# bobhansky/WhittedStyle_Raytracer

Hardware: NVIDIA B200
Metric: Mrays/s (all ray types), out/water_bunny_tex.txt + shadow soft @ 3840x2160 (higher is better)
Workload: dtype f32

## Files before the change

### include/wrt_cuda.h

```cpp
#ifndef WRT_CUDA_H
#define WRT_CUDA_H

#include "wrt_scene.h"

#ifdef __cplusplus
extern "C" {
#endif

typedef struct WrtContext WrtContext;

#define WRT_TRAVERSAL_EXHAUSTIVE 0
#define WRT_TRAVERSAL_PRUNED     1


int  wrt_create(int device, WrtContext** out);
void wrt_destroy(WrtContext* ctx);
const char* wrt_last_error(void);

int wrt_upload_scene(WrtContext* ctx, const WrtSceneDesc* scene);
int wrt_set_camera(WrtContext* ctx, const WrtCamera* cam);

int wrt_set_tiles(WrtContext* ctx, int tile_w, int tile_h, int rank, int world);

int wrt_set_options(WrtContext* ctx, int traversal, uint32_t seed, float queue_factor);

int wrt_enable_kernel_timing(WrtContext* ctx, int on);

int wrt_trace_closest(WrtContext* ctx, const float* orig, const float* dir, int64_t n, WrtHit* hits);
int wrt_trace_closest_wavefront(WrtContext* ctx, const float* orig, const float* dir, int64_t n, WrtHit* hits);
int wrt_shadow_hard(WrtContext* ctx, const float* pos, const float* ndir, const float* lightpos, int64_t n, float* coeff);
int wrt_shadow_soft(WrtContext* ctx, const float* pos, const float* ndir, const float* lightpos, int64_t n, float* coeff);
int wrt_shadow_directional(WrtContext* ctx, const float* pos, const int32_t* self_object, const float* lightdir4,
                           int64_t n, float* coeff);

int wrt_render(WrtContext* ctx, uint8_t* rgb_host, WrtStats* stats);

int wrt_render_device(WrtContext* ctx, void* d_rgb_tiles, void* cuda_stream);
int wrt_finish_device(WrtContext* ctx, WrtStats* stats);
int wrt_get_stats(WrtContext* ctx, WrtStats* stats);

int64_t wrt_tile_pixel_count(WrtContext* ctx, int rank, int world);

int wrt_scatter_tiles(WrtContext* ctx, const void* d_gathered, int world, int64_t stride_bytes,
                      void* d_rgb_image, void* cuda_stream);

int64_t wrt_kernel_launch_count(WrtContext* ctx);

int wrt_measure_fp32_peak(WrtContext* ctx, float* tflops_fma, float* tflops_mul_add);

#define WRT_KERNEL_FAMILIES 11
int wrt_get_kernel_times(WrtContext* ctx, float* ms, int capacity);
int wrt_get_kernel_launches(WrtContext* ctx, int32_t* launches, int capacity);

typedef struct WrtMulti WrtMulti;
int  wrt_multi_create(const int* devices, int n, WrtMulti** out);
void wrt_multi_destroy(WrtMulti* m);
int  wrt_multi_device_count(WrtMulti* m);
WrtContext* wrt_multi_context(WrtMulti* m, int rank);
int  wrt_multi_uses_peer_stores(WrtMulti* m);
int  wrt_multi_upload_scene(WrtMulti* m, const WrtSceneDesc* scene);
int  wrt_multi_set_camera(WrtMulti* m, const WrtCamera* cam);
int  wrt_multi_set_options(WrtMulti* m, int traversal, uint32_t seed, float queue_factor);
int  wrt_multi_render(WrtMulti* m, uint8_t* rgb_host, WrtStats* stats);

#ifdef __cplusplus
}
#endif
#endif
```

### whittedstyle_raytracer_b200/csrc/cuda/kernels.cuh

```cuda
#pragma once
#include <cooperative_groups.h>

#include "dev_shade.cuh"
#include "shaft_cull.h"
#include "../../../include/wrt_rng.h"
#include "../../../include/wrt_tiles.h"

#ifdef WRT_MIN_BLOCKS
#define WRT_TRACE_BOUNDS __launch_bounds__(128, WRT_MIN_BLOCKS)
#else
#define WRT_TRACE_BOUNDS __launch_bounds__(128)
#endif
#ifndef WRT_TRACE_DEEP_STEPS
#define WRT_TRACE_DEEP_STEPS 8
#endif
namespace wrt {

#ifdef WRT_DEBUG_BOUNDS
__device__ unsigned g_wrt_bounds_line = 0;
__device__ __forceinline__ bool wrt_bounds_ok(bool ok, unsigned line) {
    if (!ok) atomicCAS(&g_wrt_bounds_line, 0u, line);
    return ok;
}
#define WRT_IN_BOUNDS(idx, cap) wrt_bounds_ok((unsigned long long)(idx) < (unsigned long long)(cap), (unsigned)__LINE__)
#else
#define WRT_IN_BOUNDS(idx, cap) true
#endif

enum CounterSlot {
    C_NRAYS = 0,
    C_NTRAYS = 112,
    C_NPREQ = 16,
    C_NDREQ = 32,
    C_VALID0 = 48,
    C_OVERFLOW = 49,
    C_NEMPTY = 50,
    C_NCULL = 128,
    C_NSKIP = 144,
    C_NDSKIP = 160,
    C_POOL = 176,
    C_NWORK = 180,
    C_WORK = 192,
    C_TOTAL = 256
};

struct TileMap : WrtTileMap {
    __host__ __device__ bool slot_to_pixel(long long slot, int rank_, int& px, int& py) const {
        return wrt_tilemap_slot_to_pixel(this, slot, rank_, &px, &py) != 0;
    }
};

#define WRT_QUEUES 3

struct PrimaryGen {
    WrtCamera cam;
    TileMap tm;
    long long slot0;
};

struct FrameBuffers {
    float4* ray_o[2];
    float4* ray_d[2];
    float4* hit;
    float4* surf;
    float4* node_a;
    float4* node_b;
    float4* preq_o[WRT_QUEUES];
    uint4*  preq_k[WRT_QUEUES];
    float4* dreq_o[WRT_QUEUES];
    uint4*  dreq_k[WRT_QUEUES];
    unsigned char queue_of_level[WRT_MAX_DEPTH + 3];
    float*  coeff;
    unsigned* counters;
    unsigned cap0, capd;
    unsigned preq_cap[WRT_QUEUES], dreq_cap[WRT_QUEUES];
    unsigned n_node_cap;
};

__device__ __forceinline__ unsigned node_id(const FrameBuffers& fb, int level, unsigned slot) {
    return level == 0 ? slot : fb.cap0 + (unsigned)(level - 1) * fb.capd + slot;
}

__device__ __forceinline__ unsigned warp_alloc(unsigned* counter, int k, unsigned cap, unsigned* overflow) {
    unsigned lane = threadIdx.x & 31;
    int incl = k;
#pragma unroll
    for (int off = 1; off < 32; off <<= 1) {
        int n = __shfl_up_sync(0xffffffffu, incl, off);
        if (lane >= (unsigned)off) incl += n;
    }
    int total = __shfl_sync(0xffffffffu, incl, 31);
    unsigned base = 0;
    if (lane == 31 && total > 0) base = atomicAdd(counter, (unsigned)total);
    base = __shfl_sync(0xffffffffu, base, 31);
    unsigned mine = base + (unsigned)(incl - k);
    if (k > 0 && (mine > cap || (unsigned)k > cap - mine)) { *overflow = 1u; return 0xffffffffu; }
    return mine;
}

struct LevelSpan {
    unsigned nR, nT, half;
    __device__ __forceinline__ unsigned count() const { return nR + nT; }
    __device__ __forceinline__ unsigned slot(unsigned item) const { return item < nR ? item : half + (item - nR); }
};
__device__ __forceinline__ LevelSpan level_span(const FrameBuffers& fb, int level, unsigned n0) {
    LevelSpan sp;
    if (level == 0) {
        sp.half = fb.cap0; sp.nT = 0;
        sp.nR = n0 < fb.cap0 ? n0 : fb.cap0;
    } else {
        const unsigned* counters = fb.counters;
        sp.half = fb.capd / 2;
        sp.nR = counters[C_NRAYS + level] < sp.half ? counters[C_NRAYS + level] : sp.half;
        sp.nT = counters[C_NTRAYS + level] < fb.capd - sp.half ? counters[C_NTRAYS + level] : fb.capd - sp.half;
    }
    return sp;
}

__device__ __forceinline__ unsigned queue_len(const unsigned* counters, int slot, unsigned cap) {
    unsigned n = counters[slot];
    return n < cap ? n : cap;
}

__device__ __forceinline__ bool primary_ray(const PrimaryGen& pg, unsigned item, f3& org, f3& dir, unsigned& pixel) {
    const WrtCamera& cam = pg.cam;
    int x, y;
    if (!pg.tm.slot_to_pixel(pg.slot0 + item, pg.tm.rank, x, y)) {
        org = mk3(0.f, 0.f, 0.f); dir = mk3(0.f, 0.f, 1.f); pixel = 0xffffffffu;
        return false;
    }
    f3 ul = mk3(cam.ul[0], cam.ul[1], cam.ul[2]);
    f3 v_off = (float)y * mk3(cam.delta_v[0], cam.delta_v[1], cam.delta_v[2]);
    f3 h_off = (float)x * mk3(cam.delta_h[0], cam.delta_h[1], cam.delta_h[2]);
    f3 pixelPos = ul + h_off + v_off + mk3(cam.c_off_h[0], cam.c_off_h[1], cam.c_off_h[2]) +
                  mk3(cam.c_off_v[0], cam.c_off_v[1], cam.c_off_v[2]);
    f3 eye = mk3(cam.eye[0], cam.eye[1], cam.eye[2]);
    f3 nrm = mk3(cam.n[0], cam.n[1], cam.n[2]);
    if (!cam.parallel) { dir = normalized(pixelPos - eye); org = eye; }
    else { dir = nrm; org = pixelPos - cam.d * nrm; }
    pixel = (unsigned)(y * cam.width + x);
    return true;
}

#define WRT_CULL_UNLIT 1
#define WRT_CULL_SHAFT 2
__device__ __forceinline__ void surface_warp(const DevScene& s, const FrameBuffers& fb, int level, int cull, bool live,
                                             f3 org, f3 dir, unsigned pixel, unsigned path, float hit_t, int prim,
                                             float b1, float b2, unsigned slot) {
    const unsigned child_half = fb.capd / 2;
    const int q = fb.queue_of_level[level];
    float4* nray_o = fb.ray_o[(level + 1) & 1];
// ... 155 lines not shown
            unsigned pixel;
            if (!primary_ray(pg, (unsigned)item, o, d, pixel)) { cs.best.prim = -2; return false; }
        } else {
            o = mk3(ray_o[idx]); d = mk3(ray_d[idx]);
        }
        if (s.n_nodes == 0) return false;
        r = make_ray(o, d);
        float prune = prune_cfg;
        const bool ref_tree = prune < 0.f || degenerate_dir(r.d);
        if (ref_tree) prune = -1.f;
        const size_t oct_off = (size_t)ray_octant(r.d) * 2 * (size_t)s.n_nodes;
        nodes = (ref_tree ? s.ronodes : s.onodes) + oct_off;
        cs.set_ray(s, r, prune);
        float te;
        float4 lo = ldg4(nodes), hi = ldg4(nodes + 1);
        if (!slab_presorted(lo, hi, r, te)) return false;
        cur = __float_as_int(lo.w);
        if (cur < 0) { cs.leaf(s, r, ~cur); return false; }
        wide = WRT_WIDE4 && !LEVEL0 && !ref_tree;
        if (wide) nodes = s.wnodes + (WRT_WIDE_FLOAT4_PER_RECORD / 2) * oct_off;
        return true;
    }
    __device__ __forceinline__ bool step(int& cur, Stack& st) {
#if WRT_LEAF_DEFER
        if (WRT_WIDE4 && !LEVEL0 && wide) return traverse_step4_defer<true>(nodes, r, st, cur, cs.limit, [&](int p) { cs.leaf(s, r, p); });
#else
        if (WRT_WIDE4 && !LEVEL0 && wide) return traverse_step4<true>(nodes, r, st, cur, cs.limit, [&](int p) { cs.leaf(s, r, p); });
#endif
        return traverse_step<true, true>(nodes, r, st, cur, cs.limit, [&](int p) { cs.leaf(s, r, p); });
    }
    __device__ __forceinline__ bool finish(int&, Stack&) {
        if (WRT_IN_BOUNDS(idx, fb.cap0 > fb.capd ? fb.cap0 : fb.capd))
            fb.hit[idx] = make_float4(cs.best.t, __int_as_float(cs.best.prim), cs.best.u, cs.best.v);
        return false;
    }
};

template <bool LEVEL0>
__global__ void WRT_TRACE_BOUNDS k_trace_closest(const __grid_constant__ DevScene s, const __grid_constant__ FrameBuffers fb,
                                                 const __grid_constant__ PrimaryGen pg, int level, unsigned n0, int work_slot,
                                                 float prune_rel, int refill) {
    extern __shared__ int smem[];
    Stack st;
    st.init(smem, threadIdx.x, blockDim.x);
    ClosestQuery<LEVEL0> q(s, fb, pg, level, n0, prune_rel);
    run_queue<ClosestQuery<LEVEL0>, LEVEL0 ? WRT_STEPS_PER_ROUND : WRT_TRACE_DEEP_STEPS>(
        q, q.span.count(), reinterpret_cast<unsigned long long*>(fb.counters + work_slot), st, refill);
}

#ifndef WRT_SURFACE_MIN_BLOCKS
#define WRT_SURFACE_MIN_BLOCKS 4
#endif
__global__ void __launch_bounds__(256, WRT_SURFACE_MIN_BLOCKS) k_surface_spawn(const __grid_constant__ DevScene s, const __grid_constant__ FrameBuffers fb,
                                                       const __grid_constant__ PrimaryGen pg, int level, unsigned n0, int cull) {
    const LevelSpan span = level_span(fb, level, n0);
    const unsigned n = span.count();
    const unsigned n_round = (n + 31u) & ~31u;
    unsigned valid = 0;
    for (unsigned item = blockIdx.x * blockDim.x + threadIdx.x; item < n_round; item += gridDim.x * blockDim.x) {
        const bool live = item < n;
        const unsigned i = span.slot(live ? item : 0);
        f3 org = mk3(0.f, 0.f, 0.f), dir = org;
        unsigned pixel = 0, path = 0;
        float4 h = make_float4(0.f, __int_as_float(-2), 0.f, 0.f);
        if (live) {
            h = fb.hit[i];
            if (level == 0) {
                path = 1u;
                if (primary_ray(pg, item, org, dir, pixel)) ++valid;
            } else {
                float4 o4 = fb.ray_o[level & 1][i], d4 = fb.ray_d[level & 1][i];
                org = mk3(o4); dir = mk3(d4);
                pixel = __float_as_uint(o4.w); path = __float_as_uint(d4.w);
            }
        }
        surface_warp(s, fb, level, cull, live, org, dir, pixel, path, h.x, __float_as_int(h.y), h.z, h.w, i);
    }
    if (level == 0) {
        valid = __reduce_add_sync(0xffffffffu, valid);
        if ((threadIdx.x & 31) == 0 && valid) atomicAdd(fb.counters + C_VALID0, valid);
    }
}

struct HardShadowQuery {
    const DevScene& s;
    const FrameBuffers& fb;
    Ray r;
    const float4* nodes;
    float dis;
    ShadowAcc acc;
    size_t out;
    int q;
    bool wide;
    bool literal;
    __device__ __forceinline__ HardShadowQuery(const DevScene& s_, const FrameBuffers& fb_, int q_, bool literal_)
        : s(s_), fb(fb_), q(q_), literal(literal_) {}
    __device__ __forceinline__ bool begin(unsigned long long item, int& cur, Stack&) {
        float4 o4 = fb.preq_o[q][item];
        uint4 k = fb.preq_k[q][item];
        const WrtLight* L = s.lights + k.x;
        f3 orig = mk3(o4);
        f3 lightPos = mk3(L->pos[0], L->pos[1], L->pos[2]);
        f3 raydir = normalized(lightPos - orig);
        dis = norm(lightPos - orig);
        r = make_ray(orig, raydir);
        out = (size_t)__float_as_uint(o4.w) * (unsigned)s.n_lights + k.x;
        acc.reset();
        if (s.n_nodes == 0) return false;
        const bool ref_tree = literal || degenerate_dir(raydir);
        const size_t oct_off = (size_t)ray_octant(raydir) * 2 * (size_t)s.n_nodes;
        nodes = (ref_tree ? s.ronodes : s.onodes) + oct_off;
        float te;
        float4 lo = ldg4(nodes), hi = ldg4(nodes + 1);
        if (!slab_presorted(lo, hi, r, te)) return false;
        cur = __float_as_int(lo.w);
        if (cur < 0) { shadow_leaf(s, r, dis, ~cur, acc); return false; }
        wide = WRT_WIDE4 && !ref_tree;
        if (wide) nodes = s.wnodes + (WRT_WIDE_FLOAT4_PER_RECORD / 2) * oct_off;
        return true;
    }
    __device__ __forceinline__ bool step(int& cur, Stack& st) {
        const float never = INFINITY;
        bool more;
#if WRT_LEAF_DEFER >= 2
        if (WRT_WIDE4 && wide) more = traverse_step4_defer<false>(nodes, r, st, cur, never, [&](int p) { shadow_leaf(s, r, dis, p, acc); });
#else
        if (WRT_WIDE4 && wide) more = traverse_step4<false>(nodes, r, st, cur, never, [&](int p) { shadow_leaf(s, r, dis, p, acc); });
#endif
        else more = traverse_step<false, true>(nodes, r, st, cur, never, [&](int p) { shadow_leaf(s, r, dis, p, acc); });
        return more && acc.res != 0.f;
    }
    __device__ __forceinline__ bool finish(int&, Stack&) {
        const float v = shadow_value(s, acc);
        if (WRT_IN_BOUNDS(out, (size_t)fb.n_node_cap * s.n_lights)) fb.coeff[out] = v;
        return false;
    }
};

__global__ void WRT_TRACE_BOUNDS k_shadow_hard(const __grid_constant__ DevScene s, const __grid_constant__ FrameBuffers fb, int q, int work_slot, int refill,
                                               int literal) {
    extern __shared__ int smem[];
    Stack st;
    st.init(smem, threadIdx.x, blockDim.x);
    const unsigned n = queue_len(fb.counters, C_NPREQ + q, fb.preq_cap[q]);
    HardShadowQuery hq(s, fb, q, literal != 0);
    run_queue(hq, n, reinterpret_cast<unsigned long long*>(fb.counters + work_slot), st, refill);
}

struct SoftShadowQuery {
    const DevScene& s;
    const FrameBuffers& fb;
    unsigned seed;
    Ray r;
    const float4* nodes;
    float dis;
    bool occ;
    size_t out;
    int q;
    int last_occ;
    bool use_cache;
    __device__ __forceinline__ SoftShadowQuery(const DevScene& s_, const FrameBuffers& fb_, unsigned seed_, int q_, bool cache)
        : s(s_), fb(fb_), seed(seed_), q(q_), last_occ(-1), use_cache(cache && !s_.has_light_prims) {}
    __device__ __forceinline__ bool begin(unsigned long long item, int& cur, Stack& st) {
        unsigned req = (unsigned)(item / WRT_SOFT_SAMPLES);
        unsigned sample = (unsigned)(item - (unsigned long long)req * WRT_SOFT_SAMPLES);
        float4 o4 = fb.preq_o[q][req];
// ... 832 lines not shown
```

### whittedstyle_raytracer_b200/csrc/cuda/ploc_bvh.h

```cpp
#ifndef WRT_PLOC_BVH_H
#define WRT_PLOC_BVH_H

#include <math.h>
#include <stdint.h>

#ifdef __CUDACC__
#define WRT_PLOC_HD __host__ __device__ __forceinline__
#else
#include <vector_types.h>
#include <vector_functions.h>
#define WRT_PLOC_HD static inline
#endif

#define WRT_PLOC_RADIUS 8

struct PlocTree {
    float4* lo;
    float4* hi;
    float4* dlo;
    float4* dhi;
    int* parent;
    int* cnt;
};

WRT_PLOC_HD float ploc_fmin(float a, float b) { return a < b ? a : b; }
WRT_PLOC_HD float ploc_fmax(float a, float b) { return a > b ? a : b; }
WRT_PLOC_HD int ploc_f2i(float f) { union { float f; int i; } u; u.f = f; return u.i; }
WRT_PLOC_HD float ploc_i2f(int i) { union { float f; int i; } u; u.i = i; return u.f; }

WRT_PLOC_HD uint64_t ploc_expand21(uint64_t v) {
    v &= 0x1fffffull;
    v = (v | v << 32) & 0x1f00000000ffffull;
    v = (v | v << 16) & 0x1f0000ff0000ffull;
    v = (v | v << 8) & 0x100f00f00f00f00full;
    v = (v | v << 4) & 0x10c30c30c30c30c3ull;
    v = (v | v << 2) & 0x1249249249249249ull;
    return v;
}
WRT_PLOC_HD uint64_t ploc_morton(const float c[3], const float bmin[3], const float bmax[3]) {
    uint64_t code = 0;
    for (int k = 0; k < 3; k++) {
        float ext = bmax[k] - bmin[k];
        float t = ext > 0.f ? (c[k] - bmin[k]) / ext : 0.f;
        if (!(t > 0.f)) t = 0.f;
        if (t > 1.f) t = 1.f;
        uint64_t q = (uint64_t)(t * 2097151.0f);
        code |= ploc_expand21(q) << k;
    }
    return code;
}

WRT_PLOC_HD void ploc_init_leaf(const PlocTree& t, int p, const float mn[3], const float mx[3], float dil_rel, float dil_abs) {
    t.lo[p] = make_float4(mn[0], mn[1], mn[2], ploc_i2f(-1));
    t.hi[p] = make_float4(mx[0], mx[1], mx[2], ploc_i2f(-1));
    float ext = 0.f;
    for (int k = 0; k < 3; k++) {
        ext = ploc_fmax(ext, mx[k] - mn[k]);
        ext = ploc_fmax(ext, ploc_fmax(fabsf(mn[k]), fabsf(mx[k])) * 1e-2f);
    }
    const float pad = dil_rel * ext + dil_abs;
    t.dlo[p] = make_float4(mn[0] - pad, mn[1] - pad, mn[2] - pad, 0.f);
    t.dhi[p] = make_float4(mx[0] + pad, mx[1] + pad, mx[2] + pad, 0.f);
    t.parent[p] = -1;
    t.cnt[p] = 1;
}

WRT_PLOC_HD float ploc_union_area(const float4 alo, const float4 ahi, const float4 blo, const float4 bhi) {
    float dx = ploc_fmax(ahi.x, bhi.x) - ploc_fmin(alo.x, blo.x);
    float dy = ploc_fmax(ahi.y, bhi.y) - ploc_fmin(alo.y, blo.y);
    float dz = ploc_fmax(ahi.z, bhi.z) - ploc_fmin(alo.z, blo.z);
    return dx * dy + dy * dz + dz * dx;
}

WRT_PLOC_HD bool ploc_tie_before(int i, int j, int k) {
    const bool jb = j == (i ^ 1), kb = k == (i ^ 1);
    if (jb != kb) return jb;
    const int dj = j > i ? j - i : i - j, dk = k > i ? k - i : i - k;
    if (dj != dk) return dj < dk;
    return (j < i ? j : i) < (k < i ? k : i);
}
WRT_PLOC_HD int ploc_nearest(const PlocTree& t, const int* cl, int m, int i, int radius) {
    const int a = cl[i];
    const float4 alo = t.lo[a], ahi = t.hi[a];
    float best = INFINITY;
    int bj = -1;
    const int j0 = i - radius > 0 ? i - radius : 0, j1 = i + radius < m - 1 ? i + radius : m - 1;
    for (int j = j0; j <= j1; j++) {
        if (j == i) continue;
        const int b = cl[j];
        float d = ploc_union_area(alo, ahi, t.lo[b], t.hi[b]);
        if (!(d == d)) d = INFINITY;
        if (bj < 0 || d < best || (d == best && ploc_tie_before(i, j, bj))) { best = d; bj = j; }
    }
    return bj;
}

WRT_PLOC_HD int ploc_fate(const int* nn, int i) {
    const int j = nn[i];
    if (j < 0 || nn[j] != i) return 1;
    return i < j ? 2 : 0;
}

WRT_PLOC_HD void ploc_make_node(const PlocTree& t, int id, int a, int b) {
    const float4 alo = t.lo[a], ahi = t.hi[a], blo = t.lo[b], bhi = t.hi[b];
    t.lo[id] = make_float4(ploc_fmin(alo.x, blo.x), ploc_fmin(alo.y, blo.y), ploc_fmin(alo.z, blo.z), ploc_i2f(a));
    t.hi[id] = make_float4(ploc_fmax(ahi.x, bhi.x), ploc_fmax(ahi.y, bhi.y), ploc_fmax(ahi.z, bhi.z), ploc_i2f(b));
    const float4 dal = t.dlo[a], dah = t.dhi[a], dbl = t.dlo[b], dbh = t.dhi[b];
    t.dlo[id] = make_float4(ploc_fmin(dal.x, dbl.x), ploc_fmin(dal.y, dbl.y), ploc_fmin(dal.z, dbl.z), 0.f);
    t.dhi[id] = make_float4(ploc_fmax(dah.x, dbh.x), ploc_fmax(dah.y, dbh.y), ploc_fmax(dah.z, dbh.z), 0.f);
    t.cnt[id] = t.cnt[a] + t.cnt[b];
    t.parent[id] = -1;
    t.parent[a] = id;
    t.parent[b] = id;
}

WRT_PLOC_HD int ploc_record_of(const PlocTree& t, int n_leaves, int v, int* link, int* depth) {
    int acc = 0, d = 0, own_extra = 0, own_right = 0;
    int u = v;
    while (t.parent[u] >= 0) {
        const int p = t.parent[u];
        const int left = ploc_f2i(t.lo[p].w);
        const int right = u != left;
        const int extra = 2 + (right ? 2 * t.cnt[left] - 2 : 0);
        if (u == v) { own_extra = extra; own_right = right; }
        acc += extra;
        u = p;
        ++d;
    }
    *depth = d;
    const int F = 2 + acc;
    *link = v < n_leaves ? ~v : F;
    return d == 0 ? 0 : F - own_extra + own_right;
// ... 4 lines not shown
```

### whittedstyle_raytracer_b200/csrc/cuda/wrt_cuda.cu

```cuda
#include <algorithm>
#include <cstdio>
#include <chrono>
#include <cstdlib>
#include <cstring>
#include <condition_variable>
#include <functional>
#include <mutex>
#include <string>
#include <thread>
#include <vector>

#include <cuda_runtime.h>

#include "../../../include/wrt_cuda.h"
#include "fast_bvh.hpp"
#include "kernels.cuh"
#include "bvh_build.cuh"

namespace {

thread_local std::string g_err;

int fail(const std::string& msg) {
    g_err = msg;
    return 1;
}

#define CK(call)                                                                                      \
    do {                                                                                              \
        cudaError_t e_ = (call);                                                                      \
        if (e_ != cudaSuccess) {                                                                      \
            return fail(std::string(#call) + ": " + cudaGetErrorString(e_) + " (" + __FILE__ + ":" + \
                        std::to_string(__LINE__) + ")");                                              \
        }                                                                                             \
    } while (0)

enum Family { F_RAYGEN, F_TRACE, F_SURFACE, F_SHADOW_HARD, F_SHADOW_SOFT, F_SHADOW_DIR, F_SHADE, F_COMBINE, F_RESOLVE, F_SOFT_LISTS, F_SOFT_FILTER };

struct TimedLaunch {
    int family;
    cudaEvent_t e0, e1;
    bool on_chain;
};

}

struct WrtContext {
    int device = 0;
    int num_sms = 0;
    cudaStream_t chain = nullptr, side = nullptr;
    cudaEvent_t ev_in = nullptr, ev_lvl0 = nullptr, ev_mid = nullptr, ev_side = nullptr, ev_out = nullptr;
    bool overlap = true;

    wrt::DevScene ds{};
    std::vector<void*> scene_allocs;
    std::vector<size_t> scene_alloc_bytes;
    size_t scene_slot = 0;
    bool has_scene = false;
    bool textures_complete = true;
    int bvh_depth = 0;
    int stack_rows = 2;
    std::vector<WrtPathCode> path_codes;

    WrtCamera cam{};
    bool has_cam = false;
    int tile_w = 8, tile_h = 4, rank = 0, world = 1;
    int traversal = WRT_TRAVERSAL_PRUNED;
    uint32_t seed = WRT_DEFAULT_SEED;
    float queue_factor = 0.f;
    float deep_factor = 0.25f;
    float prune_rel = 1e-3f;
    bool kernel_timing = false;
    int refill = 16;
    int refill_soft = 24;
    bool shaft_cull = true;
    bool soft_lists = true;
    long long list_pool_cap_override = 0;
    int shaft_cull_max_level = 0;
    wrt::SoftListBuffers list_bufs[WRT_QUEUES] = {};
    wrt::FastBvhBuilder fbvh;
    bool host_bvh = false;
    uint8_t* h_stage = nullptr;
    size_t h_stage_bytes = 0;
    int ploc_coop_grid = 1;
    int fast_depth = 0, build_passes = 0;
    bool unlit_cull = true;
    int cache_from_level = 0;
    int chunk_div = 16;
    int refill0 = 32;
    int trace_blocks_per_sm = 10;
    bool shade0_separate = true;
    int soft_filter = 2;
    int deep_split = 5;
    int side_blocks_per_sm = 6;
    int fb_split = -1;
    bool small_batch_full_levels = true;
    long long max_batch = 1ll << 25;
    long long learned_batch = 1ll << 40;
    long long learned_key[4] = {0, 0, 0, 0};

    wrt::FrameBuffers fb{};
    std::vector<void*> frame_allocs;
    unsigned batch_slots = 0;
    unsigned deep_slots = 0;
    int fb_lights = -1, fb_point = -1, fb_dir = -1;
    unsigned* h_counters = nullptr;
    uint8_t* d_image = nullptr;
    size_t d_image_bytes = 0;
    uint8_t* h_image = nullptr;
    size_t h_image_bytes = 0;

    void* d_scratch[5] = {nullptr, nullptr, nullptr, nullptr, nullptr};
    size_t scratch_bytes[5] = {0, 0, 0, 0, 0};

    int64_t launches = 0;
    int work_seq = 0;
    int coop_grid = 0;
    int filter_grid = 0;
    WrtStats stats{};
    std::vector<TimedLaunch> timed;
    std::vector<cudaEvent_t> event_pool;
    size_t event_next = 0;
    float family_ms[WRT_KERNEL_FAMILIES] = {0};
    int family_launches[WRT_KERNEL_FAMILIES] = {0};
    cudaEvent_t ev_begin = nullptr, ev_end = nullptr;
    cudaStream_t user_stream = nullptr;
    bool user_stream_joined = false;
    uint8_t* last_image = nullptr;
    uint8_t* last_packed = nullptr;
    bool frame_pending = false;
    bool has_frame = false;

    wrt::TileMap tilemap() const {
        wrt::TileMap tm;
        static_cast<WrtTileMap&>(tm) = wrt_tilemap_make(cam.width, cam.height, tile_w, tile_h, rank, world);
        return tm;
    }
    long long local_slots(int r, int w) const {
        WrtTileMap tm = wrt_tilemap_make(cam.width, cam.height, tile_w, tile_h, r, w);
        return wrt_tilemap_slots(&tm, r, w);
    }
};

namespace {

using wrt::FrameBuffers;

int dev_alloc(WrtContext* c, size_t bytes, void** out) {
    *out = nullptr;
    bytes = std::max<size_t>(bytes, 256);
    size_t slot = c->scene_slot++;
    if (slot >= c->scene_allocs.size()) { c->scene_allocs.push_back(nullptr); c->scene_alloc_bytes.push_back(0); }
    if (c->scene_alloc_bytes[slot] < bytes) {
        if (c->scene_allocs[slot]) {
            CK(cudaDeviceSynchronize());
            cudaFree(c->scene_allocs[slot]);
        }
        c->scene_allocs[slot] = nullptr; c->scene_alloc_bytes[slot] = 0;
        CK(cudaMalloc(&c->scene_allocs[slot], bytes));
        c->scene_alloc_bytes[slot] = bytes;
    }
// ... 6 lines not shown
    c->scene_allocs.clear();
    c->scene_alloc_bytes.clear();
    c->has_scene = false;
}

void free_frame(WrtContext* c) {
    for (void* p : c->frame_allocs) cudaFree(p);
    c->frame_allocs.clear();
    c->batch_slots = 0;
    c->deep_slots = 0;
    memset(&c->fb, 0, sizeof c->fb);
}

int tree_depth(const WrtSceneDesc* s) {
    if (s->n_nodes == 0) return 0;
    int maxd = 0;
    std::vector<std::pair<int, int>> st;
    st.push_back({0, 0});
    while (!st.empty()) {
        auto [n, d] = st.back();
        st.pop_back();
        maxd = std::max(maxd, d);
        int link = s->nodes[n].link;
        if (link >= 0) { st.push_back({link, d + 1}); st.push_back({link + 1, d + 1}); }
    }
    return maxd;
}

template <class T>
int frame_alloc(WrtContext* c, T** p, size_t count) {
    void* q = nullptr;
    CK(cudaMalloc(&q, std::max<size_t>(count, 1) * sizeof(T)));
    c->frame_allocs.push_back(q);
    *p = (T*)q;
    return 0;
}

unsigned deep_slots_for(const WrtContext* c, unsigned slots) {
    double want;
    if (c->queue_factor > 0.f) want = (double)slots * c->queue_factor;
    else want = std::max((double)slots * c->deep_factor, c->small_batch_full_levels ? std::min((double)slots, 1048576.0) : 0.0);
    want = std::min(want, 2.0e9);
    return ((unsigned)std::max(want, 64.0) + 63u) & ~63u;
}

int ensure_frame_buffers(WrtContext* c, unsigned slots) {
    const wrt::DevScene& ds = c->ds;
    const unsigned capd = deep_slots_for(c, slots);
    if (c->batch_slots >= slots && c->deep_slots >= capd && c->fb_lights == ds.n_lights && c->fb_point == ds.n_point_lights &&
        c->fb_dir == ds.n_dir_lights && c->fb_split == c->deep_split)
        return 0;
    CK(cudaDeviceSynchronize());
    free_frame(c);
    FrameBuffers& fb = c->fb;
    const unsigned cap0 = slots + 64;
    const unsigned long long nodes64 = (unsigned long long)cap0 + (unsigned long long)(WRT_MAX_DEPTH - 1) * capd;
    if (nodes64 > 0x7fffff00ull) return fail("frame batch too large for 32-bit node indices");
    if (nodes64 * std::max(1, ds.n_lights) > 0xffffffffffull) return fail("too many (node, light) pairs");
    fb.cap0 = cap0; fb.capd = capd; fb.n_node_cap = (unsigned)nodes64;
    const unsigned long long deep_nodes = (unsigned long long)(WRT_MAX_DEPTH - 1) * capd;
    auto req_cap = [](unsigned long long nodes, int lights) {
        return (unsigned)std::min<unsigned long long>(nodes * (unsigned long long)std::max(1, lights), 0xffffff00ull);
    };
    (void)deep_nodes;
    const int split = std::max(1, std::min(WRT_MAX_DEPTH - 1, c->deep_split));
    const unsigned long long q_nodes[WRT_QUEUES] = {cap0, (unsigned long long)split * capd, (unsigned long long)(WRT_MAX_DEPTH - 1 - split) * capd};
    for (int q = 0; q < WRT_QUEUES; q++) {
        fb.preq_cap[q] = req_cap(std::max(q_nodes[q], 1ull), ds.n_point_lights);
        fb.dreq_cap[q] = req_cap(std::max(q_nodes[q], 1ull), ds.n_dir_lights);
    }
    for (int d = 0; d < WRT_MAX_DEPTH; d++) fb.queue_of_level[d] = (unsigned char)(d == 0 ? 0 : (d <= split ? 1 : 2));
    for (int k = 0; k < 2; k++) {
        if (frame_alloc(c, &fb.ray_o[k], capd)) return 1;
        if (frame_alloc(c, &fb.ray_d[k], capd)) return 1;
    }
    if (frame_alloc(c, &fb.hit, std::max(cap0, capd))) return 1;
    if (frame_alloc(c, &fb.surf, 4 * (size_t)nodes64)) return 1;
    if (frame_alloc(c, &fb.node_a, (size_t)nodes64)) return 1;
    if (frame_alloc(c, &fb.node_b, (size_t)nodes64)) return 1;
    if (frame_alloc(c, &fb.coeff, (size_t)nodes64 * std::max(1, ds.n_lights))) return 1;
    for (int q = 0; q < WRT_QUEUES; q++) {
        if (frame_alloc(c, &fb.preq_o[q], ds.n_point_lights ? fb.preq_cap[q] : 1)) return 1;
        if (frame_alloc(c, &fb.preq_k[q], ds.n_point_lights ? fb.preq_cap[q] : 1)) return 1;
        if (frame_alloc(c, &fb.dreq_o[q], ds.n_dir_lights ? fb.dreq_cap[q] : 1)) return 1;
        if (frame_alloc(c, &fb.dreq_k[q], ds.n_dir_lights ? fb.dreq_cap[q] : 1)) return 1;
    }
    if (frame_alloc(c, &fb.counters, wrt::C_TOTAL)) return 1;
    for (int q = 0; q < WRT_QUEUES; q++) {
        wrt::SoftListBuffers& lb = c->list_bufs[q];
        lb.region_per_request = q == 0 ? 4u : 32u;
        const unsigned long long per_req = q == 0 ? 4ull : 16ull;
        lb.pool_cap = (unsigned)std::min<unsigned long long>(std::max<unsigned long long>(8ull << 20, per_req * fb.preq_cap[q]), 1ull << 30);
        if (!ds.n_point_lights || ds.shadow_type == 0) lb.pool_cap = 64;
        if (c->list_pool_cap_override > 0) lb.pool_cap = (unsigned)c->list_pool_cap_override;
        const bool lists_possible = ds.n_point_lights && ds.shadow_type != 0;
        if (frame_alloc(c, &lb.scratch, lists_possible ? (size_t)c->num_sms * c->trace_blocks_per_sm * 128 * WRT_LIST_CAP : 1)) return 1;
        if (frame_alloc(c, &lb.shafts, lists_possible ? (size_t)c->num_sms * c->trace_blocks_per_sm * 4 * WRT_LISTS_CHUNK * WRT_SHAFT_SLOT : 1)) return 1;
        if (frame_alloc(c, &lb.pool, lb.pool_cap)) return 1;
        if (frame_alloc(c, &lb.ref, lists_possible ? fb.preq_cap[q] : 1)) return 1;
        if (frame_alloc(c, &lb.work, lists_possible ? fb.preq_cap[q] : 1)) return 1;
    }
    c->batch_slots = slots;
    c->deep_slots = capd;
    c->fb_lights = ds.n_lights; c->fb_point = ds.n_point_lights; c->fb_dir = ds.n_dir_lights;
    c->fb_split = c->deep_split;
    return 0;
}

int ensure_scratch(WrtContext* c, int k, size_t bytes) {
    if (c->scratch_bytes[k] >= bytes) return 0;
    if (c->d_scratch[k]) cudaFree(c->d_scratch[k]);
    c->d_scratch[k] = nullptr;
    c->scratch_bytes[k] = 0;
    CK(cudaMalloc(&c->d_scratch[k], bytes));
    c->scratch_bytes[k] = bytes;
    return 0;
}

cudaEvent_t next_event(WrtContext* c) {
    if (c->event_next == c->event_pool.size()) {
        cudaEvent_t e;
        cudaEventCreate(&e);
        c->event_pool.push_back(e);
    }
    return c->event_pool[c->event_next++];
}

struct LaunchScope {
    WrtContext* c;
    cudaStream_t st;
    TimedLaunch tl{};
    bool timed;
    LaunchScope(WrtContext* ctx, cudaStream_t s, int family) : c(ctx), st(s), timed(ctx->kernel_timing) {
        ++c->launches;
        if (timed) {
            tl.family = family;
            tl.on_chain = s == ctx->chain;
            tl.e0 = next_event(c);
            tl.e1 = next_event(c);
            cudaEventRecord(tl.e0, st);
        }
    }
    ~LaunchScope() {
        if (timed) {
            cudaEventRecord(tl.e1, st);
            c->timed.push_back(tl);
        }
    }
};

int grid_for(WrtContext* c, int blocks_per_sm) { return c->num_sms * blocks_per_sm; }

size_t stack_bytes(WrtContext* c, int threads) { return (size_t)c->stack_rows * threads * sizeof(int); }

float prune_value(const WrtContext* c) { return c->traversal == WRT_TRAVERSAL_PRUNED ? c->prune_rel : -1.f; }

int enqueue_shadows(WrtContext* c, cudaStream_t st, int q, int& work_seq) {
    using namespace wrt;
    FrameBuffers& fb = c->fb;
    const DevScene& ds = c->ds;
    const int TB = 128;
    const bool on_side = st == c->side && c->side_blocks_per_sm > 0;
    const int trace_grid = grid_for(c, on_side ? std::min(c->side_blocks_per_sm, c->trace_blocks_per_sm) : c->trace_blocks_per_sm), wide_grid = grid_for(c, 8);
    const size_t sb = stack_bytes(c, TB);
    auto work_slot = [&]() { int s = C_WORK + 2 * work_seq; ++work_seq; return s; };
    const int refill = (q == 0 ? c->refill0 : c->refill) | (c->chunk_div << 8);
    if (ds.n_point_lights > 0) {
        if (ds.shadow_type == 0) {
            LaunchScope ls(c, st, F_SHADOW_HARD);
            k_shadow_hard<<<trace_grid, TB, sb, st>>>(ds, fb, q, work_slot(), refill, c->traversal == WRT_TRAVERSAL_EXHAUSTIVE ? 1 : 0);
        } else {
            const bool lists = c->soft_lists && !ds.has_light_prims && ds.n_nodes > 0 && c->traversal == WRT_TRAVERSAL_PRUNED &&
                               (unsigned long long)fb.preq_cap[q] * WRT_SOFT_SAMPLES < (1ull << 32);
            if (lists) {
                const SoftListBuffers& lb = c->list_bufs[q];
                {
                    LaunchScope ls(c, st, F_SOFT_LISTS);
                    k_soft_lists<<<trace_grid, TB, sb, st>>>(ds, fb, q, work_slot(), c->stack_rows, lb);
                }
                const bool filtered = c->soft_filter >= (q == 0 ? 2 : 1);
                if (filtered) {
                    LaunchScope ls(c, st, F_SOFT_FILTER);
                    k_soft_filter<<<WRT_FILTER_DYNAMIC ? c->filter_grid : wide_grid, TB, 0, st>>>(ds, fb, q, lb, WRT_FILTER_DYNAMIC ? work_slot() : 0);
                }
                LaunchScope ls(c, st, F_SHADOW_SOFT);
                k_soft_list_rays<<<trace_grid, TB, sb, st>>>(ds, fb, q, work_slot(), c->seed, lb, filtered ? 1 : 0);
            } else {
                LaunchScope ls(c, st, F_SHADOW_SOFT);
                k_shadow_soft<<<trace_grid, TB, sb, st>>>(ds, fb, q, work_slot(), c->seed, c->refill_soft | (c->chunk_div << 8),
                                                          c->cache_from_level <= (q == 0 ? 0 : 1) ? 1 : 0);
            }
        }
    }
    if (ds.n_dir_lights > 0) {
        LaunchScope ls(c, st, F_SHADOW_DIR);
        k_shadow_directional<<<wide_grid, TB, sb, st>>>(ds, fb, q, c->traversal == WRT_TRAVERSAL_EXHAUSTIVE ? 1 : 0);
    }
    return 0;
}

int enqueue_batch(WrtContext* c, long long slot0, unsigned n, uint8_t* d_image, uint8_t* d_packed) {
    using namespace wrt;
    FrameBuffers& fb = c->fb;
    const DevScene& ds = c->ds;
    cudaStream_t st = c->chain;
    const bool overlap = c->overlap && (!c->kernel_timing || getenv("WRT_TIMING_OVERLAP") != nullptr);
    cudaStream_t ss = overlap ? c->side : st;
    PrimaryGen pg;
    pg.cam = c->cam; pg.tm = c->tilemap(); pg.slot0 = slot0;
    CK(cudaMemsetAsync(fb.counters, 0, C_TOTAL * sizeof(unsigned), st));
    int work_seq = 0;
    auto work_slot = [&]() { int s = C_WORK + 2 * work_seq; ++work_seq; return s; };
    const int TB = 128;
    const int trace_grid = grid_for(c, c->trace_blocks_per_sm), wide_grid = grid_for(c, 8);
    const size_t sb = stack_bytes(c, TB);
    const float prune = prune_value(c);
    auto cull_for = [&](int d) {
        int cull = 0;
        if (c->traversal == WRT_TRAVERSAL_PRUNED) {
            if (c->unlit_cull) cull |= WRT_CULL_UNLIT;
            const bool lists_on = c->soft_lists && !ds.has_light_prims;
            if (c->shaft_cull && ds.shadow_type != 0 && (d <= c->shaft_cull_max_level || !lists_on)) cull |= WRT_CULL_SHAFT;
        }
        return cull;
    };
    auto level_kernels = [&](int d) {
        const int refill = (d == 0 ? c->refill0 : c->refill) | (c->chunk_div << 8);
        {
            LaunchScope ls(c, st, F_TRACE);
            if (d == 0) k_trace_closest<true><<<trace_grid, TB, sb, st>>>(ds, fb, pg, d, n, work_slot(), prune, refill);
            else k_trace_closest<false><<<trace_grid, TB, sb, st>>>(ds, fb, pg, d, n, work_slot(), prune, refill);
        }
        LaunchScope ls(c, st, F_SURFACE);
        k_surface_spawn<<<wide_grid, 256, 0, st>>>(ds, fb, pg, d, n, cull_for(d));
    };
    level_kernels(0);
    if (overlap) {
        CK(cudaEventRecord(c->ev_lvl0, st));
        CK(cudaStreamWaitEvent(ss, c->ev_lvl0, 0));
    }
    if (enqueue_shadows(c, ss, 0, work_seq)) return 1;
    if (c->shade0_separate) {
        LaunchScope ls(c, ss, F_SHADE);
        k_shade<<<wide_grid, 256, 0, ss>>>(ds, fb, n, 0, 0);
    }
    const int split = std::max(1, std::min(WRT_MAX_DEPTH - 1, c->deep_split));
    for (int d = 1; d <= split; d++) level_kernels(d);
    if (overlap) {
        CK(cudaEventRecord(c->ev_mid, st));
        CK(cudaStreamWaitEvent(ss, c->ev_mid, 0));
    }
    if (enqueue_shadows(c, ss, 1, work_seq)) return 1;
    if (overlap) CK(cudaEventRecord(c->ev_side, ss));
    for (int d = split + 1; d < WRT_MAX_DEPTH; d++) level_kernels(d);
    if (split < WRT_MAX_DEPTH - 1 && enqueue_shadows(c, st, 2, work_seq)) return 1;
    if (overlap) CK(cudaStreamWaitEvent(st, c->ev_side, 0));
    {
        LaunchScope ls(c, st, F_COMBINE);
// ... 159 lines not shown
    }
    if (check_debug_bounds()) return 1;
    float ms = 0.f;
    if (cudaEventElapsedTime(&ms, c->ev_begin, c->ev_end) == cudaSuccess) c->stats.gpu_ms = ms;
    for (float& f : c->family_ms) f = 0.f;
    for (int& n : c->family_launches) n = 0;
    const bool dump = getenv("WRT_TIMING_DUMP") != nullptr;
    for (const TimedLaunch& tl : c->timed) {
        float t = 0.f;
        if (cudaEventElapsedTime(&t, tl.e0, tl.e1) == cudaSuccess) { c->family_ms[tl.family] += t; ++c->family_launches[tl.family]; }
        if (dump) {
            float t0 = 0.f, t1 = 0.f;
            cudaEventElapsedTime(&t0, c->ev_begin, tl.e0);
            cudaEventElapsedTime(&t1, c->ev_begin, tl.e1);
            fprintf(stderr, "[wrt] launch family %d: %.1f us  (%s stream, %.1f -> %.1f us after the frame's start)\n", tl.family, t * 1e3f,
                    tl.on_chain ? "chain" : "side", t0 * 1e3f, t1 * 1e3f);
        }
    }
    return 0;
}

}

extern "C" {

const char* wrt_last_error(void) { return g_err.c_str(); }

int wrt_create(int device, WrtContext** out) {
    if (!out) return fail("wrt_create: null out pointer");
    *out = nullptr;
    int n = 0;
    cudaError_t e = cudaGetDeviceCount(&n);
    if (e != cudaSuccess || n == 0)
        return fail(std::string("wrt_create: no CUDA device (") + cudaGetErrorString(e) +
                    "); this library has no CPU fallback");
    if (device < 0 || device >= n) return fail("wrt_create: device index out of range");
    CK(cudaSetDevice(device));
    cudaDeviceProp prop;
    CK(cudaGetDeviceProperties(&prop, device));
    if (prop.major < 10)
        return fail(std::string("wrt_create: ") + prop.name + " is sm_" + std::to_string(prop.major) +
                    std::to_string(prop.minor) + "; this library is built for sm_100a only");
    WrtContext* c = new WrtContext();
    c->device = device;
    c->num_sms = prop.multiProcessorCount;
    int prio_least = 0, prio_greatest = 0;
    cudaDeviceGetStreamPriorityRange(&prio_least, &prio_greatest);
    bool ev_ok = cudaStreamCreateWithPriority(&c->chain, cudaStreamNonBlocking, prio_greatest) == cudaSuccess &&
                 cudaStreamCreateWithPriority(&c->side, cudaStreamNonBlocking, prio_least) == cudaSuccess;
    for (cudaEvent_t* e : {&c->ev_in, &c->ev_lvl0, &c->ev_mid, &c->ev_side, &c->ev_out})
        ev_ok = ev_ok && cudaEventCreateWithFlags(e, cudaEventDisableTiming) == cudaSuccess;
    if (!ev_ok ||
        cudaEventCreate(&c->ev_begin) != cudaSuccess || cudaEventCreate(&c->ev_end) != cudaSuccess ||
        cudaMallocHost((void**)&c->h_counters, (wrt::C_TOTAL + 64) * sizeof(unsigned)) != cudaSuccess) {
        delete c;
        return fail("wrt_create: stream/event/pinned allocation failed");
    }
    memset(c->h_counters, 0, wrt::C_TOTAL * sizeof(unsigned));
    {
        int per_sm = 0;
        if (cudaOccupancyMaxActiveBlocksPerMultiprocessor(&per_sm, wrt::k_combine_resolve, 256, 0) != cudaSuccess || per_sm < 1) {
            wrt_destroy(c);
            return fail("wrt_create: cooperative launch of k_combine_resolve is not possible on this device");
        }
        c->coop_grid = c->num_sms * std::min(per_sm, 4);
        per_sm = 0;
        if (cudaOccupancyMaxActiveBlocksPerMultiprocessor(&per_sm, wrt::k_bvh_ploc, WRT_PLOC_THREADS, 0) != cudaSuccess || per_sm < 1) {
            wrt_destroy(c);
            return fail("wrt_create: cooperative launch of k_bvh_ploc is not possible on this device");
        }
        c->ploc_coop_grid = c->num_sms * std::min(per_sm, 2);
        per_sm = 0;
        if (cudaOccupancyMaxActiveBlocksPerMultiprocessor(&per_sm, wrt::k_soft_filter, 128, 0) != cudaSuccess || per_sm < 1) per_sm = 4;
        c->filter_grid = c->num_sms * per_sm;
    }
    if (const char* e = getenv("WRT_REFILL")) c->refill = std::max(1, std::min(32, atoi(e)));
    if (const char* e = getenv("WRT_REFILL_SOFT")) c->refill_soft = std::max(1, std::min(32, atoi(e)));
    if (const char* e = getenv("WRT_TRACE_BLOCKS")) c->trace_blocks_per_sm = std::max(1, std::min(32, atoi(e)));
    if (const char* e = getenv("WRT_OVERLAP")) c->overlap = atoi(e) != 0;
    if (const char* e = getenv("WRT_CACHE_FROM")) c->cache_from_level = atoi(e);
    if (const char* e = getenv("WRT_SHAFT_CULL")) c->shaft_cull = atoi(e) != 0;
    if (const char* e = getenv("WRT_UNLIT_CULL")) c->unlit_cull = atoi(e) != 0;
    if (const char* e = getenv("WRT_SOFT_LISTS")) c->soft_lists = atoi(e) != 0;
    if (const char* e = getenv("WRT_LIST_POOL_CAP")) c->list_pool_cap_override = atoll(e);
    if (const char* e = getenv("WRT_SHAFT_LEVELS")) c->shaft_cull_max_level = atoi(e);
    if (const char* e = getenv("WRT_CHUNK_DIV")) c->chunk_div = std::max(0, std::min(255, atoi(e)));
    if (const char* e = getenv("WRT_REFILL0")) c->refill0 = std::max(1, std::min(32, atoi(e)));
    if (const char* e = getenv("WRT_HOST_BVH")) c->host_bvh = atoi(e) != 0;
    if (const char* e = getenv("WRT_SHADE0_SEPARATE")) c->shade0_separate = atoi(e) != 0;
    if (const char* e = getenv("WRT_SOFT_FILTER")) c->soft_filter = atoi(e);
    if (const char* e = getenv("WRT_SIDE_BLOCKS")) c->side_blocks_per_sm = std::max(0, std::min(32, atoi(e)));
    if (const char* e = getenv("WRT_DEEP_SPLIT")) c->deep_split = std::max(1, std::min(WRT_MAX_DEPTH - 1, atoi(e)));
    if (const char* e = getenv("WRT_DEEP_FACTOR")) { c->deep_factor = std::max(0.001f, std::min(2.f, (float)atof(e))); c->small_batch_full_levels = false; }
    if (const char* e = getenv("WRT_MAX_BATCH")) c->max_batch = std::max(64ll, (atoll(e) + 31) / 32 * 32);
    *out = c;
    return 0;
}

void wrt_destroy(WrtContext* c) {
    if (!c) return;
    cudaSetDevice(c->device);
    cudaDeviceSynchronize();
    free_scene(c);
    free_frame(c);
    for (int k = 0; k < 5; k++) if (c->d_scratch[k]) cudaFree(c->d_scratch[k]);
    if (c->d_image) cudaFree(c->d_image);
    if (c->h_image) cudaFreeHost(c->h_image);
    if (c->h_counters) cudaFreeHost(c->h_counters);
    if (c->h_stage) cudaFreeHost(c->h_stage);
    for (cudaEvent_t e : c->event_pool) cudaEventDestroy(e);
    if (c->ev_begin) cudaEventDestroy(c->ev_begin);
    if (c->ev_end) cudaEventDestroy(c->ev_end);
    for (cudaEvent_t e : {c->ev_in, c->ev_lvl0, c->ev_mid, c->ev_side, c->ev_out}) if (e) cudaEventDestroy(e);
    if (c->side) cudaStreamDestroy(c->side);
    if (c->chain) cudaStreamDestroy(c->chain);
    delete c;
}

int wrt_upload_scene(WrtContext* c, const WrtSceneDesc* s) {
    if (!c || !s) return fail("wrt_upload_scene: null argument");
    CK(cudaSetDevice(c->device));
    if (s->n_nodes < 0 || s->n_prims < 0 || s->n_materials < 0 || s->n_lights < 0 || s->n_textures < 0 || s->n_normalmaps < 0 || s->n_texels < 0)
        return fail("wrt_upload_scene: negative count in the scene description");
    if (s->n_prims > 0 && s->n_nodes != 2 * s->n_prims)
        return fail("wrt_upload_scene: a tree over n one-primitive leaves has 2n records (root, padding, n-1 sibling pairs)");
    if (s->n_prims > 0 && s->n_materials == 0) return fail("wrt_upload_scene: primitives without materials");
    for (int i = 0; i < s->n_textures + s->n_normalmaps; i++) {
        const WrtTexture& t = i < s->n_textures ? s->textures[i] : s->normalmaps[i - s->n_textures];
        if (t.offset < 0 || t.count < 0 || t.offset + t.count > s->n_texels) return fail("wrt_upload_scene: texture texel range outside texels[]");
    }
    for (int i = 0; i < s->n_nodes; i++) {
        const int link = s->nodes[i].link;
        if (i != 1 && link >= 0 && (link < 2 || link + 1 >= s->n_nodes)) return fail("wrt_upload_scene: tree child link out of range");
    }
    cudaStream_t st = c->chain;
    c->has_scene = false;
    c->scene_slot = 0;
    wrt::DevScene& ds = c->ds;
    memset(&ds, 0, sizeof ds);
    c->textures_complete = true;
    const int np = s->n_prims, nn = s->n_nodes;
    static_assert(sizeof(WrtNode) == 32, "WrtNode must be 32 bytes");
    static_assert(sizeof(WrtMaterial) == 48, "WrtMaterial must be 12 floats");

    c->bvh_depth = tree_depth(s);

    struct Part { const void* src; size_t bytes; size_t off; };
    Part parts[] = {
        {s->nodes, (size_t)nn * sizeof(WrtNode), 0},
        {s->prim_geom, (size_t)np * 48, 0},
        {s->prim_flags, (size_t)np * 4, 0},
        {s->prim_material, (size_t)np * 4, 0},
        {s->prim_texture, (size_t)np * 4, 0},
        {s->prim_normalmap, (size_t)np * 4, 0},
        {s->prim_object, (size_t)np * 4, 0},
        {s->object_prim, (size_t)np * 4, 0},
        {s->prim_normals, (size_t)np * 36, 0},
        {s->prim_uv, (size_t)np * 24, 0},
        {s->materials, (size_t)s->n_materials * sizeof(WrtMaterial), 0},
        {s->lights, (size_t)s->n_lights * sizeof(WrtLight), 0},
        {s->textures, (size_t)s->n_textures * sizeof(WrtTexture), 0},
        {s->normalmaps, (size_t)s->n_normalmaps * sizeof(WrtTexture), 0},
        {s->texels, (size_t)s->n_texels * 12, 0},
        {nullptr, 0, 0},
    };
    if (wrt_make_path_codes(s->nodes, nn, np, c->path_codes)) {
// ... 710 lines not shown
```

### whittedstyle_raytracer_b200/renderer.py

```python
from __future__ import annotations

import ctypes as C

import numpy as np

from . import cabi
from .scene import Scene

TRAVERSAL_EXHAUSTIVE = 0
TRAVERSAL_PRUNED = 1

KERNEL_FAMILIES = ["raygen", "trace_closest", "surface", "shadow_hard", "shadow_soft", "shadow_directional",
                   "shade", "combine", "resolve", "soft_lists", "soft_filter"]


class CudaError(RuntimeError):
    pass


def _f32(a, cols):
    a = np.ascontiguousarray(a, dtype=np.float32)
    if a.ndim != 2 or a.shape[1] != cols:
        raise ValueError(f"expected an (N, {cols}) float array, got {a.shape}")
    return a


def stats_dict(st: cabi.WrtStats) -> dict:
    return {
        "closest_rays": int(st.closest_rays), "shadow_rays": int(st.shadow_rays),
        "rays": int(st.closest_rays + st.shadow_rays),
        "rays_per_depth": [int(x) for x in st.rays_per_depth],
        "shadow_requests": int(st.shadow_requests), "overflow_retries": int(st.overflow_retries),
        "gpu_ms": float(st.gpu_ms),
        "shaft_culled_requests": int(st.shaft_culled_requests),
        "unlit_skipped_requests": int(st.unlit_skipped_requests),
        "shadow_rays_traced": int(st.shadow_rays_traced),
    }


class Context:

    def __init__(self, device: int = 0):
        self.lib = cabi.load_cuda()
        self.h = C.c_void_p()
        self._check(self.lib.wrt_create(device, C.byref(self.h)))
        self.scene = None

    def _check(self, rc):
        if rc != 0:
            raise CudaError(self.lib.wrt_last_error().decode(errors="replace"))

    def close(self):
        if getattr(self, "h", None):
            self.lib.wrt_destroy(self.h)
            self.h = C.c_void_p()

    def __del__(self):
        try:
            self.close()
        except Exception:
            pass

    def upload_scene(self, scene: Scene):
        self._check(self.lib.wrt_upload_scene(self.h, scene.desc_ptr))
        self._check(self.lib.wrt_set_camera(self.h, scene.camera_ptr))
        self.scene = scene

    def set_camera(self, scene: Scene):
        self._check(self.lib.wrt_set_camera(self.h, scene.camera_ptr))

    def set_tiles(self, tile_w=8, tile_h=4, rank=0, world=1):
        self._check(self.lib.wrt_set_tiles(self.h, tile_w, tile_h, rank, world))

    def set_options(self, traversal=TRAVERSAL_PRUNED, seed=cabi.WRT_DEFAULT_SEED, queue_factor=0.0):
        self._check(self.lib.wrt_set_options(self.h, traversal, seed, queue_factor))

    def enable_kernel_timing(self, on=True):
        self._check(self.lib.wrt_enable_kernel_timing(self.h, 1 if on else 0))

    @property
    def launches(self) -> int:
        return int(self.lib.wrt_kernel_launch_count(self.h))

    def kernel_times(self) -> dict:
        ms = (C.c_float * len(KERNEL_FAMILIES))()
        n = self.lib.wrt_get_kernel_times(self.h, ms, len(KERNEL_FAMILIES))
        return {KERNEL_FAMILIES[i]: float(ms[i]) for i in range(n)}

    def kernel_launches(self) -> dict:
        n = (C.c_int32 * len(KERNEL_FAMILIES))()
        k = self.lib.wrt_get_kernel_launches(self.h, n, len(KERNEL_FAMILIES))
        return {KERNEL_FAMILIES[i]: int(n[i]) for i in range(k)}

    def measure_fp32_peak(self) -> tuple[float, float]:
        a, b = C.c_float(0), C.c_float(0)
        self._check(self.lib.wrt_measure_fp32_peak(self.h, C.byref(a), C.byref(b)))
# ... 123 lines not shown
```

Before: 7119.

## Sort secondary shadow requests by light and Morton origin before traversal

Adds a kernel that radix-sorts the point-light shadow requests of secondary queues within 4096-item tiles. The sort key packs the light index above a Morton code of the ray origin, and the sorted requests are copied into new buffers that the shadow kernels then read. The goal is more coherent BVH traversal and memory access in the hard and soft shadow kernels. In exchange it adds an extra launch, extra buffers, and a gather pass over every request in each of those queues.

```diff
diff --git a/include/wrt_cuda.h b/include/wrt_cuda.h
--- a/include/wrt_cuda.h
+++ b/include/wrt_cuda.h
@@ -48,7 +48,7 @@
 
 int wrt_measure_fp32_peak(WrtContext* ctx, float* tflops_fma, float* tflops_mul_add);
 
-#define WRT_KERNEL_FAMILIES 11
+#define WRT_KERNEL_FAMILIES 12
 int wrt_get_kernel_times(WrtContext* ctx, float* ms, int capacity);
 int wrt_get_kernel_launches(WrtContext* ctx, int32_t* launches, int capacity);
 
diff --git a/whittedstyle_raytracer_b200/csrc/cuda/kernels.cuh b/whittedstyle_raytracer_b200/csrc/cuda/kernels.cuh
--- a/whittedstyle_raytracer_b200/csrc/cuda/kernels.cuh
+++ b/whittedstyle_raytracer_b200/csrc/cuda/kernels.cuh
@@ -1,8 +1,10 @@
 #pragma once
 #include <cooperative_groups.h>
+#include <cub/block/block_radix_sort.cuh>
 
 #include "dev_shade.cuh"
 #include "shaft_cull.h"
+#include "ploc_bvh.h"
 #include "../../../include/wrt_rng.h"
 #include "../../../include/wrt_tiles.h"
 
@@ -67,6 +69,8 @@
     float4* node_b;
     float4* preq_o[WRT_QUEUES];
     uint4*  preq_k[WRT_QUEUES];
+    float4* preq_so[WRT_QUEUES];
+    uint4*  preq_sk[WRT_QUEUES];
     float4* dreq_o[WRT_QUEUES];
     uint4*  dreq_k[WRT_QUEUES];
     unsigned char queue_of_level[WRT_MAX_DEPTH + 3];
@@ -388,6 +392,48 @@
     }
 }
 
+#ifndef WRT_ORDER_TILE
+#define WRT_ORDER_TILE 4096
+#endif
+#define WRT_ORDER_THREADS 256
+__global__ void __launch_bounds__(WRT_ORDER_THREADS) k_order_requests(const __grid_constant__ DevScene s, const __grid_constant__ FrameBuffers fb, int q) {
+    constexpr int ITEMS = WRT_ORDER_TILE / WRT_ORDER_THREADS;
+    using Sort = cub::BlockRadixSort<unsigned, WRT_ORDER_THREADS, ITEMS, unsigned>;
+    __shared__ typename Sort::TempStorage tmp;
+    const unsigned n = queue_len(fb.counters, C_NPREQ + q, fb.preq_cap[q]);
+    float bmin[3] = {0.f, 0.f, 0.f}, bmax[3] = {0.f, 0.f, 0.f};
+    if (s.n_nodes > 0) {
+        const float4 lo = ldg4(s.onodes), hi = ldg4(s.onodes + 1);
+        bmin[0] = lo.x; bmin[1] = lo.y; bmin[2] = lo.z;
+        bmax[0] = hi.x; bmax[1] = hi.y; bmax[2] = hi.z;
+    }
+    const int light_bits = wrt_request_key_light_bits(s.n_lights);
+    for (unsigned long long t0 = (unsigned long long)blockIdx.x * WRT_ORDER_TILE; t0 < n; t0 += (unsigned long long)gridDim.x * WRT_ORDER_TILE) {
+        unsigned key[ITEMS], val[ITEMS];
+#pragma unroll
+        for (int j = 0; j < ITEMS; j++) {
+            const unsigned long long i = t0 + threadIdx.x * ITEMS + (unsigned)j;
+            key[j] = 0xffffffffu; val[j] = 0xffffffffu;
+            if (i < n) {
+                const float4 o4 = fb.preq_o[q][i];
+                const float o[3] = {o4.x, o4.y, o4.z};
+                key[j] = wrt_request_key(o, bmin, bmax, fb.preq_k[q][i].x, light_bits);
+                val[j] = (unsigned)i;
+            }
+        }
+        Sort(tmp).SortBlockedToStriped(key, val);
+#pragma unroll
+        for (int j = 0; j < ITEMS; j++) {
+            const unsigned long long i = t0 + (unsigned)j * WRT_ORDER_THREADS + threadIdx.x;
+            if (i < n && WRT_IN_BOUNDS(i, fb.preq_cap[q]) && WRT_IN_BOUNDS(val[j], fb.preq_cap[q])) {
+                fb.preq_so[q][i] = fb.preq_o[q][val[j]];
+                fb.preq_sk[q][i] = fb.preq_k[q][val[j]];
+            }
+        }
+        __syncthreads();
+    }
+}
+
 struct HardShadowQuery {
     const DevScene& s;
     const FrameBuffers& fb;
diff --git a/whittedstyle_raytracer_b200/csrc/cuda/ploc_bvh.h b/whittedstyle_raytracer_b200/csrc/cuda/ploc_bvh.h
--- a/whittedstyle_raytracer_b200/csrc/cuda/ploc_bvh.h
+++ b/whittedstyle_raytracer_b200/csrc/cuda/ploc_bvh.h
@@ -48,6 +48,28 @@
         code |= ploc_expand21(q) << k;
     }
     return code;
+}
+
+WRT_PLOC_HD int wrt_request_key_light_bits(int n_lights) {
+    int b = 0;
+    while (b < 32 && (1ll << b) < (long long)n_lights) ++b;
+    return b;
+}
+WRT_PLOC_HD uint32_t wrt_request_key(const float o[3], const float bmin[3], const float bmax[3], unsigned light, int light_bits) {
+    int bits = (32 - light_bits) / 3;
+    if (bits > 10) bits = 10;
+    const float scale = (float)((1u << bits) - 1u);
+    uint64_t code = 0;
+    for (int k = 0; k < 3; k++) {
+        const float ext = bmax[k] - bmin[k];
+        float t = ext > 0.f ? (o[k] - bmin[k]) / ext : 0.f;
+        if (!(t > 0.f)) t = 0.f;
+        if (t > 1.f) t = 1.f;
+        code |= ploc_expand21((uint64_t)(t * scale)) << k;
+    }
+    const int free_bits = 32 - light_bits;
+    const uint32_t morton = (uint32_t)code << (free_bits - 3 * bits);
+    return light_bits > 0 ? ((uint32_t)light << free_bits) | morton : morton;
 }
 
 WRT_PLOC_HD void ploc_init_leaf(const PlocTree& t, int p, const float mn[3], const float mx[3], float dil_rel, float dil_abs) {
diff --git a/whittedstyle_raytracer_b200/csrc/cuda/wrt_cuda.cu b/whittedstyle_raytracer_b200/csrc/cuda/wrt_cuda.cu
--- a/whittedstyle_raytracer_b200/csrc/cuda/wrt_cuda.cu
+++ b/whittedstyle_raytracer_b200/csrc/cuda/wrt_cuda.cu
@@ -35,7 +35,7 @@
         }                                                                                             \
     } while (0)
 
-enum Family { F_RAYGEN, F_TRACE, F_SURFACE, F_SHADOW_HARD, F_SHADOW_SOFT, F_SHADOW_DIR, F_SHADE, F_COMBINE, F_RESOLVE, F_SOFT_LISTS, F_SOFT_FILTER };
+enum Family { F_RAYGEN, F_TRACE, F_SURFACE, F_SHADOW_HARD, F_SHADOW_SOFT, F_SHADOW_DIR, F_SHADE, F_COMBINE, F_RESOLVE, F_SOFT_LISTS, F_SOFT_FILTER, F_ORDER };
 
 struct TimedLaunch {
     int family;
@@ -77,6 +77,7 @@
     bool soft_lists = true;
     long long list_pool_cap_override = 0;
     int shaft_cull_max_level = 0;
+    bool sort_requests = true;
     wrt::SoftListBuffers list_bufs[WRT_QUEUES] = {};
     wrt::FastBvhBuilder fbvh;
     bool host_bvh = false;
@@ -249,6 +250,11 @@
     for (int q = 0; q < WRT_QUEUES; q++) {
         if (frame_alloc(c, &fb.preq_o[q], ds.n_point_lights ? fb.preq_cap[q] : 1)) return 1;
         if (frame_alloc(c, &fb.preq_k[q], ds.n_point_lights ? fb.preq_cap[q] : 1)) return 1;
+        fb.preq_so[q] = nullptr; fb.preq_sk[q] = nullptr;
+        if (ds.n_point_lights && q > 0 && c->sort_requests) {
+            if (frame_alloc(c, &fb.preq_so[q], fb.preq_cap[q])) return 1;
+            if (frame_alloc(c, &fb.preq_sk[q], fb.preq_cap[q])) return 1;
+        }
         if (frame_alloc(c, &fb.dreq_o[q], ds.n_dir_lights ? fb.dreq_cap[q] : 1)) return 1;
         if (frame_alloc(c, &fb.dreq_k[q], ds.n_dir_lights ? fb.dreq_cap[q] : 1)) return 1;
     }
@@ -324,7 +330,7 @@
 
 int enqueue_shadows(WrtContext* c, cudaStream_t st, int q, int& work_seq) {
     using namespace wrt;
-    FrameBuffers& fb = c->fb;
+    FrameBuffers fb = c->fb;
     const DevScene& ds = c->ds;
     const int TB = 128;
     const bool on_side = st == c->side && c->side_blocks_per_sm > 0;
@@ -332,8 +338,17 @@
     const size_t sb = stack_bytes(c, TB);
     auto work_slot = [&]() { int s = C_WORK + 2 * work_seq; ++work_seq; return s; };
     const int refill = (q == 0 ? c->refill0 : c->refill) | (c->chunk_div << 8);
+    auto order_requests = [&]() {
+        if (!fb.preq_so[q]) return;
+        LaunchScope ls(c, st, F_ORDER);
+        const unsigned tiles = (unsigned)(((unsigned long long)fb.preq_cap[q] + WRT_ORDER_TILE - 1) / WRT_ORDER_TILE);
+        k_order_requests<<<std::min(tiles, (unsigned)grid_for(c, 4)), WRT_ORDER_THREADS, 0, st>>>(ds, fb, q);
+        fb.preq_o[q] = fb.preq_so[q];
+        fb.preq_k[q] = fb.preq_sk[q];
+    };
     if (ds.n_point_lights > 0) {
         if (ds.shadow_type == 0) {
+            order_requests();
             LaunchScope ls(c, st, F_SHADOW_HARD);
             k_shadow_hard<<<trace_grid, TB, sb, st>>>(ds, fb, q, work_slot(), refill, c->traversal == WRT_TRAVERSAL_EXHAUSTIVE ? 1 : 0);
         } else {
@@ -341,6 +356,7 @@
                                (unsigned long long)fb.preq_cap[q] * WRT_SOFT_SAMPLES < (1ull << 32);
             if (lists) {
                 const SoftListBuffers& lb = c->list_bufs[q];
+                order_requests();
                 {
                     LaunchScope ls(c, st, F_SOFT_LISTS);
                     k_soft_lists<<<trace_grid, TB, sb, st>>>(ds, fb, q, work_slot(), c->stack_rows, lb);
@@ -666,6 +682,7 @@
     if (const char* e = getenv("WRT_SHAFT_CULL")) c->shaft_cull = atoi(e) != 0;
     if (const char* e = getenv("WRT_UNLIT_CULL")) c->unlit_cull = atoi(e) != 0;
     if (const char* e = getenv("WRT_SOFT_LISTS")) c->soft_lists = atoi(e) != 0;
+    if (const char* e = getenv("WRT_SORT_REQUESTS")) c->sort_requests = atoi(e) != 0;
     if (const char* e = getenv("WRT_LIST_POOL_CAP")) c->list_pool_cap_override = atoll(e);
     if (const char* e = getenv("WRT_SHAFT_LEVELS")) c->shaft_cull_max_level = atoi(e);
     if (const char* e = getenv("WRT_CHUNK_DIV")) c->chunk_div = std::max(0, std::min(255, atoi(e)));
diff --git a/whittedstyle_raytracer_b200/renderer.py b/whittedstyle_raytracer_b200/renderer.py
--- a/whittedstyle_raytracer_b200/renderer.py
+++ b/whittedstyle_raytracer_b200/renderer.py
@@ -11,7 +11,7 @@
 TRAVERSAL_PRUNED = 1
 
 KERNEL_FAMILIES = ["raygen", "trace_closest", "surface", "shadow_hard", "shadow_soft", "shadow_directional",
-                   "shade", "combine", "resolve", "soft_lists", "soft_filter"]
+                   "shade", "combine", "resolve", "soft_lists", "soft_filter", "order_requests"]
 
 
 class CudaError(RuntimeError):
```

Result: no change. 7166 (median of 6 runs) (+0.7%).
